# kfirc1503/generative-audio

Hardware: AMD Instinct MI355X
Metric: spectrogram-frames/sec, NPPC K=5 FullSubNet+ train step (higher is better)
Workload: dtype bf16

## Files before the change

generative-audio_amd/csrc/mfma_tile.h:

```cpp
#pragma once
#include "common.h"

enum { EPI_PLAIN = 0, EPI_PRELU_STATS = 1, EPI_RESIDUAL = 2, EPI_RELU = 3, EPI_PLAIN_F32 = 4, EPI_MASK_POS = 5, EPI_RESIDUAL_GN = 6 };

struct GemmArgs {
  const void* A; long lda; long strideA;
  const void* B; long ldb; long strideB;
  void* C; long ldc; long strideC;
  const float* bias; long strideBias;
  const void* res; long ldres; long strideRes;
  const float* slope; long strideSlope;
  double* stats; long strideStats;
  int R, N, K;
  int Tp, Tv;
  int Nv;
  int relu_in;
  int ksplit;
  const float* gnv; long strideGnv;
  double gcnt; float geps;
  int staged;
  float* colpart; long strideColpart;
};

struct ConvArgs {
// ... 61 lines not shown
    f[0] = lo.x; f[1] = lo.y; f[2] = lo.z; f[3] = lo.w; f[4] = hi.x; f[5] = hi.y; f[6] = hi.z; f[7] = hi.w;
    return f;
  }
}

template <typename T, int BN> struct NtStage {
  u32x4 a0, a1, a2, a3, b0, b1, b2, b3;
  __device__ __forceinline__ void load(const T* pa, long lda, const T* pb, long ldb) {
    a0 = *reinterpret_cast<const u32x4*>(pa);
    a1 = *reinterpret_cast<const u32x4*>(pa + 32 * lda);
    a2 = *reinterpret_cast<const u32x4*>(pa + 64 * lda);
    a3 = *reinterpret_cast<const u32x4*>(pa + 96 * lda);
    b0 = *reinterpret_cast<const u32x4*>(pb);
    b1 = *reinterpret_cast<const u32x4*>(pb + 32 * ldb);
    if constexpr (BN == 128) {
      b2 = *reinterpret_cast<const u32x4*>(pb + 64 * ldb);
      b3 = *reinterpret_cast<const u32x4*>(pb + 96 * ldb);
    }
  }
  __device__ __forceinline__ void store(unsigned char* p) const {
    *reinterpret_cast<u32x4*>(p) = a0;
    *reinterpret_cast<u32x4*>(p + 32 * 128) = a1;
    *reinterpret_cast<u32x4*>(p + 64 * 128) = a2;
    *reinterpret_cast<u32x4*>(p + 96 * 128) = a3;
    *reinterpret_cast<u32x4*>(p + 128 * 128) = b0;
    *reinterpret_cast<u32x4*>(p + 128 * 128 + 32 * 128) = b1;
    if constexpr (BN == 128) {
      *reinterpret_cast<u32x4*>(p + 128 * 128 + 64 * 128) = b2;
      *reinterpret_cast<u32x4*>(p + 128 * 128 + 96 * 128) = b3;
    }
  }
};

template <typename T, int BN, typename I, typename AOf, typename BOf>
__device__ __forceinline__ void nt_lds_mainloop(f32x4 (&acc)[4][BN / 32], unsigned char* lds, I nstage, long lda, long ldb,
                                                AOf a_of, BOf b_of, int relu_in) {
  typedef typename Frag<T>::type frag;
  constexpr int KS = (128 / (int)sizeof(T)) / 32;
  constexpr int NJ = BN / 32;
  constexpr int STAGE = (128 + BN) * 128;
  const int tid = threadIdx.x, lane = tid & 63, wave = tid >> 6, n = lane & 15, q = lane >> 4;
  const int wm = wave >> 1, wn = wave & 1;
  const int srow = tid >> 3, sc = tid & 7;
  const int soff = srow * 128 + ((sc ^ (srow & 7)) << 4);
  NtStage<T, BN> st;
#pragma unroll
  for (int i = 0; i < 4; ++i)
#pragma unroll
    for (int j = 0; j < NJ; ++j) acc[i][j] = f32x4{0.f, 0.f, 0.f, 0.f};
  {
    const T* pa = a_of((I)0);
    st.load(pa, lda, b_of((I)0), ldb);
  }
  st.store(lds + soff);
  __syncthreads();
  for (I s = 0; s < nstage; ++s) {
    const int buf = (int)(s & 1);
    const unsigned char* ta = lds + buf * STAGE;
    if (s + 1 < nstage) {
      const T* pa = a_of(s + 1);
      st.load(pa, lda, b_of(s + 1), ldb);
    }
#pragma unroll
    for (int ks = 0; ks < KS; ++ks) {
      frag af[4], bf[NJ];
#pragma unroll
      for (int i = 0; i < 4; ++i) {
        af[i] = lds_frag<T>(ta, wm * 64 + 16 * i + n, ks, q);
        if (relu_in) af[i] = relu_frag<T>(af[i]);
      }
#pragma unroll
      for (int j = 0; j < NJ; ++j) bf[j] = lds_frag<T>(ta + 128 * 128, wn * (BN / 2) + 16 * j + n, ks, q);
#pragma unroll
      for (int i = 0; i < 4; ++i)
#pragma unroll
        for (int j = 0; j < NJ; ++j) acc[i][j] = mma16(af[i], bf[j], acc[i][j]);
    }
    if (s + 1 < nstage) st.store(lds + (buf ^ 1) * STAGE + soff);
    __syncthreads();
  }
}

template <typename T, typename AOf, typename BOf>
__device__ __forceinline__ void nt_reg_mainloop(f32x4 (&acc)[2][4], int nk, long lda, long ldb, AOf a_of, BOf b_of, int relu_in) {
  typedef typename Frag<T>::type frag;
#pragma unroll
  for (int mi = 0; mi < 2; ++mi)
#pragma unroll
    for (int ni = 0; ni < 4; ++ni) acc[mi][ni] = f32x4{0.f, 0.f, 0.f, 0.f};
  frag a0[2], b0[4], a1[2], b1[4];
  auto ld = [&](frag(&a)[2], frag(&b)[4], int kk) {
    const T* pa = a_of(kk);
    const T* pb = b_of(kk);
#pragma unroll
    for (int mi = 0; mi < 2; ++mi) a[mi] = load_frag<T>(pa + (long)16 * mi * lda);
#pragma unroll
    for (int ni = 0; ni < 4; ++ni) b[ni] = load_frag<T>(pb + (long)16 * ni * ldb);
  };
  auto mm = [&](frag(&a)[2], frag(&b)[4]) {
    if (relu_in) {
#pragma unroll
      for (int mi = 0; mi < 2; ++mi) a[mi] = relu_frag<T>(a[mi]);
    }
#pragma unroll
    for (int mi = 0; mi < 2; ++mi)
#pragma unroll
      for (int ni = 0; ni < 4; ++ni) acc[mi][ni] = mma16(a[mi], b[ni], acc[mi][ni]);
  };
  ld(a0, b0, 0);
  int kk = 0;
#pragma unroll 1
  for (; kk + 2 < nk; kk += 2) {
// ... 5 lines not shown
  if (kk + 1 < nk) {
    ld(a1, b1, kk + 1);
    mm(a0, b0);
    mm(a1, b1);
  } else {
    mm(a0, b0);
  }
}

template <typename T, int EPI> struct NtEpilogue {
  const GemmArgs& g;
  const float* bias;
  const float* gnv = nullptr;
  const T* res = nullptr;
  T* C;
  float* Cf;
  float slope = 0.f, gn_rstd = 1.f, gn_mr = 0.f;
  __device__ __forceinline__ NtEpilogue(const GemmArgs& g_, int z, int m0) : g(g_) {
    C = reinterpret_cast<T*>(g.C) + (size_t)blockIdx.z * g.strideC;
    Cf = reinterpret_cast<float*>(g.C) + (size_t)blockIdx.z * g.strideC;
    bias = g.bias ? g.bias + (size_t)z * g.strideBias : nullptr;
    if (EPI == EPI_PRELU_STATS) slope = g.slope[(size_t)z * g.strideSlope];
    if (EPI == EPI_RESIDUAL_GN) {
      const double* st = g.stats + (size_t)z * g.strideStats + (size_t)(m0 / g.Tp) * 2;
      const double m = st[0] / g.gcnt, var = st[1] / g.gcnt - m * m;
      gn_rstd = (float)(1.0 / sqrt((var > 0 ? var : 0) + (double)g.geps));
      gn_mr = (float)m * gn_rstd;
      gnv = g.gnv + (size_t)z * g.strideGnv;
    }
    if (EPI == EPI_RESIDUAL || EPI == EPI_RESIDUAL_GN || EPI == EPI_MASK_POS) res = reinterpret_cast<const T*>(g.res) + (size_t)z * g.strideRes;
  }
  __device__ __forceinline__ float col_bias(int col) const {
    const bool cvalid = col < g.Nv;
    float bv = (bias && cvalid) ? bias[col] : 0.f;
    if (EPI == EPI_RESIDUAL_GN && cvalid) bv -= gn_mr * gnv[col];
    return bv;
  }
  __device__ __forceinline__ float act(float a, float bv) const {
    float v = (EPI == EPI_RESIDUAL_GN ? gn_rstd * a : a) + bv;
    if (EPI == EPI_PRELU_STATS) v = v > 0.f ? v : slope * v;
    if (EPI == EPI_RELU) v = fmaxf(v, 0.f);
    return v;
  }
  __device__ __forceinline__ float put(float a, float bv, int row, int col) const {
    const bool valid = col < g.Nv && (row % g.Tp) < g.Tv;
    float v = act(a, bv);
    if (EPI == EPI_RESIDUAL || EPI == EPI_RESIDUAL_GN) v += to_f32<T>(res[(size_t)row * g.ldres + col]);
    if (EPI == EPI_MASK_POS) {
      if (!(to_f32<T>(res[(size_t)row * g.ldres + col]) > 0.f)) v = 0.f;
    }
    if (!valid) v = 0.f;
    if (EPI == EPI_PLAIN_F32) {
      Cf[(size_t)row * g.ldc + col] = v;
      return v;
    }
    const T o = from_f32<T>(v);
    C[(size_t)row * g.ldc + col] = o;
    return to_f32<T>(o);
  }
};

__device__ __forceinline__ float mul_unfused(float a, float b) {
#pragma clang fp contract(off)
  return a * b;
}


template <typename T, int MI, int NJ>
__device__ __forceinline__ void conv_epilogue(const ConvArgs& g, const f32x4 (&acc)[MI][NJ], long row0, int col0, float (&st1)[NJ],
                                              float (&st2)[NJ]) {
  T* C = reinterpret_cast<T*>(g.C);
#pragma unroll
  for (int i = 0; i < MI; ++i)
#pragma unroll
    for (int r = 0; r < 4; ++r) {
      const long row = row0 + 16 * i + r;
      if (!interior(row, g.P, g.H, g.W)) continue;
#pragma unroll
// ... 45 lines not shown
```

generative-audio_amd/csrc/tcn.hip:

```cpp
#include <cstdlib>
#include "common.h"
#include "mfma_tile.h"
#include "nppc_hip.h"

namespace {


template <typename T, int EPI>
__global__ __launch_bounds__(256) void gemm_nt_kernel(GemmArgs g) {
  const int ks = g.ksplit > 1 ? g.ksplit : 1;
  const int z = blockIdx.z / ks, ksl = blockIdx.z % ks;
  const T* A = reinterpret_cast<const T*>(g.A) + (size_t)z * g.strideA + (size_t)ksl * g.K;
  const T* B = reinterpret_cast<const T*>(g.B) + (size_t)z * g.strideB + (size_t)ksl * g.K;
  const int lane = threadIdx.x & 63, wave = threadIdx.x >> 6, n = lane & 15, q = lane >> 4;
  const int r0 = blockIdx.x * 128 + wave * 32, c0 = blockIdx.y * 64;
  const T* ap = A + (size_t)(r0 + n) * g.lda + 8 * q;
  const T* bp = B + (size_t)(c0 + n) * g.ldb + 8 * q;
  f32x4 acc[2][4];
  nt_reg_mainloop<T>(acc, g.K / 32, g.lda, g.ldb, [&](int kk) { return ap + 32 * kk; }, [&](int kk) { return bp + 32 * kk; },
                     g.relu_in);

  const NtEpilogue<T, EPI> ep(g, z, blockIdx.x * 128);
  float s1 = 0.f, s2 = 0.f;
#pragma unroll
  for (int ni = 0; ni < 4; ++ni) {
    const int col = c0 + 16 * ni + n;
    const float bv = ep.col_bias(col);
#pragma unroll
    for (int mi = 0; mi < 2; ++mi)
#pragma unroll
      for (int j = 0; j < 4; ++j) {
        const float vo = ep.put(acc[mi][ni][j], bv, r0 + 16 * mi + 4 * q + j, col);
        if (EPI == EPI_PRELU_STATS) {
          s1 += vo;
          s2 += vo * vo;
        }
      }
  }
  if (EPI == EPI_PRELU_STATS) {
    double d1 = wave_sum((double)s1), d2 = wave_sum((double)s2);
    if (lane == 0) {
      double* st = g.stats + (size_t)z * g.strideStats + (size_t)(r0 / g.Tp) * 2;
      atomicAdd(st, d1);
      atomicAdd(st + 1, d2);
    }
  }
}

template <typename T, int EPI, int BN>
__global__ __launch_bounds__(256, 2) void gemm_nt_lds_kernel(GemmArgs g) {
  constexpr int EPC = 16 / (int)sizeof(T);
  constexpr int BK = 8 * EPC;
  constexpr int NJ = BN / 32;
  __shared__ __attribute__((aligned(16))) unsigned char lds[2][(128 + BN) * 128];
  __shared__ double red[2][4];
  const int ks_ = g.ksplit > 1 ? g.ksplit : 1;
  const int z = blockIdx.z / ks_, ksl = blockIdx.z % ks_;
  const int tid = threadIdx.x, lane = tid & 63, wave = tid >> 6, n = lane & 15, q = lane >> 4;
  const int wm = wave >> 1, wn = wave & 1;
  const int m0 = blockIdx.x * 128, n0 = blockIdx.y * BN;
  const int srow = tid >> 3, sc = tid & 7;
  const T* ga = reinterpret_cast<const T*>(g.A) + (size_t)z * g.strideA + (size_t)ksl * g.K + (long)(m0 + srow) * g.lda + sc * EPC;
  const T* gb = reinterpret_cast<const T*>(g.B) + (size_t)z * g.strideB + (size_t)ksl * g.K + (long)(n0 + srow) * g.ldb + sc * EPC;
  const int nstage = g.K / BK;
  f32x4 acc[4][NJ];
  nt_lds_mainloop<T, BN>(acc, &lds[0][0], nstage, g.lda, g.ldb, [&](int s) { return ga + s * BK; }, [&](int s) { return gb + s * BK; },
                         g.relu_in);
  const NtEpilogue<T, EPI> ep(g, z, m0);
  constexpr bool HAS_RES = EPI == EPI_RESIDUAL || EPI == EPI_RESIDUAL_GN || EPI == EPI_MASK_POS;
  constexpr bool STAGED_PLAIN = sizeof(T) == 2 && (EPI == EPI_PLAIN || EPI == EPI_PRELU_STATS || EPI == EPI_RELU);
  if constexpr (HAS_RES || STAGED_PLAIN) {
    if (g.staged) {
      constexpr int LD = BN + 4, VE = 8, CPR = BN / VE;
      constexpr int HALVES = (128 * LD * 4 <= (int)sizeof(lds)) ? 1 : 2;
      constexpr int ROWS = 128 / HALVES;
      float* ot = reinterpret_cast<float*>(&lds[0][0]);
      float csum[VE];
      float t1 = 0.f, t2 = 0.f;
#pragma unroll
      for (int e = 0; e < VE; ++e) csum[e] = 0.f;
      for (int h = 0; h < HALVES; ++h) {
        if (HALVES == 1 || wm == h) {
#pragma unroll
          for (int j = 0; j < NJ; ++j) {
            const int col = n0 + wn * (BN / 2) + 16 * j + n;
            const bool cvalid = col < g.Nv;
            const float bv = ep.col_bias(col);
#pragma unroll
            for (int i = 0; i < 4; ++i)
#pragma unroll
              for (int r = 0; r < 4; ++r) {
                const float pv = ep.act(acc[i][j][r], bv);
                ot[((HALVES == 1 ? wm * 64 : 0) + 16 * i + 4 * q + r) * LD + wn * (BN / 2) + 16 * j + n] = pv;
                if (EPI == EPI_PRELU_STATS) {
                  const int row = m0 + wm * 64 + 16 * i + 4 * q + r;
                  const float vo = (cvalid && (row % g.Tp) < g.Tv) ? to_f32<T>(from_f32<T>(pv)) : 0.f;
                  t1 += vo;
                  t2 += vo * vo;
                }
              }
          }
        }
        __syncthreads();
        for (int c = tid; c < ROWS * CPR; c += 256) {
          const int rl = c / CPR, cc = (c % CPR) * VE;
          const int row = m0 + h * ROWS * (HALVES - 1) + rl, col = n0 + cc;
          const bool rvalid = (row % g.Tp) < g.Tv;
          float v[VE], rv[VE];
          const float4 lo = *reinterpret_cast<const float4*>(ot + rl * LD + cc), hi = *reinterpret_cast<const float4*>(ot + rl * LD + cc + 4);
          v[0] = lo.x; v[1] = lo.y; v[2] = lo.z; v[3] = lo.w; v[4] = hi.x; v[5] = hi.y; v[6] = hi.z; v[7] = hi.w;
          if constexpr (HAS_RES) load8<T>(ep.res + (size_t)row * g.ldres + col, rv);
#pragma unroll
          for (int e = 0; e < VE; ++e) {
            float x = v[e];
            if constexpr (HAS_RES) {
              if (EPI == EPI_MASK_POS) { if (!(rv[e] > 0.f)) x = 0.f; }
              else x += rv[e];
            }
            if (!(rvalid && col + e < g.Nv)) x = 0.f;
            v[e] = x;
            csum[e] += to_f32<T>(from_f32<T>(x));
          }
          store8<T>(reinterpret_cast<T*>(g.C) + (size_t)blockIdx.z * g.strideC + (size_t)row * g.ldc + col, v);
        }
        if (HALVES == 2) __syncthreads();
      }
      if (EPI == EPI_PRELU_STATS) {
        const double d1 = wave_sum((double)t1), d2 = wave_sum((double)t2);
        __syncthreads();
        if (lane == 0) { red[0][wave] = d1; red[1][wave] = d2; }
        __syncthreads();
        if (tid == 0) {
          double* st = g.stats + (size_t)z * g.strideStats + (size_t)(m0 / g.Tp) * 2;
          atomicAdd(st, red[0][0] + red[0][1] + red[0][2] + red[0][3]);
          atomicAdd(st + 1, red[1][0] + red[1][1] + red[1][2] + red[1][3]);
        }
      }
      if (HAS_RES && EPI != EPI_RESIDUAL_GN && g.colpart) {
        __shared__ float cpl[4][BN];
#pragma unroll
        for (int e = 0; e < VE; ++e) {
          float cv = csum[e];
#pragma unroll
          for (int m = CPR; m < 64; m <<= 1) cv += __shfl_xor(cv, m);
          if (lane < CPR) cpl[wave][lane * VE + e] = cv;
        }
        __syncthreads();
        if (tid < BN)
          g.colpart[(size_t)z * g.strideColpart + (size_t)blockIdx.x * g.N + n0 + tid] =
              cpl[0][tid] + cpl[1][tid] + cpl[2][tid] + cpl[3][tid];
      }
      return;
    }
  }
  float s1 = 0.f, s2 = 0.f;
  float cs[NJ];
#pragma unroll
  for (int j = 0; j < NJ; ++j) {
    cs[j] = 0.f;
    const int col = n0 + wn * (BN / 2) + 16 * j + n;
    const float bv = ep.col_bias(col);
#pragma unroll
    for (int i = 0; i < 4; ++i)
#pragma unroll
      for (int r = 0; r < 4; ++r) {
        const float vo = ep.put(acc[i][j][r], bv, m0 + wm * 64 + 16 * i + 4 * q + r, col);
        if (EPI == EPI_RESIDUAL || EPI == EPI_MASK_POS) cs[j] += vo;
        if (EPI == EPI_PRELU_STATS) {
          s1 += vo;
          s2 += vo * vo;
        }
      }
  }
  if constexpr (EPI == EPI_RESIDUAL || EPI == EPI_MASK_POS) {
    if (g.colpart) {
      __shared__ float cpl[2][BN];
#pragma unroll
      for (int j = 0; j < NJ; ++j) {
        float c = cs[j];
        c += __shfl_xor(c, 16);
        c += __shfl_xor(c, 32);
        if (q == 0) cpl[wm][wn * (BN / 2) + 16 * j + n] = c;
      }
      __syncthreads();
      if (tid < BN)
        g.colpart[(size_t)z * g.strideColpart + (size_t)blockIdx.x * g.N + n0 + tid] = cpl[0][tid] + cpl[1][tid];
    }
  }
  if (EPI == EPI_PRELU_STATS) {
    const double d1 = wave_sum((double)s1), d2 = wave_sum((double)s2);
    if (lane == 0) { red[0][wave] = d1; red[1][wave] = d2; }
    __syncthreads();
    if (tid == 0) {
      double* st = g.stats + (size_t)z * g.strideStats + (size_t)(m0 / g.Tp) * 2;
      atomicAdd(st, red[0][0] + red[0][1] + red[0][2] + red[0][3]);
      atomicAdd(st + 1, red[1][0] + red[1][1] + red[1][2] + red[1][3]);
    }
  }
}
// ... 127 lines not shown
  float su = 0.f, sv = 0.f;
  for (int k = threadIdx.x; k < ldd; k += 64) {
    float wg = 0.f;
    if (nn < N && k < K) {
      const float w = W[so + (size_t)nn * K + k];
      wg = gamma[so + k] * w;
      su += beta[so + k] * w;
    }
    const T o = from_f32<T>(wg);
    dst[k] = o;
    sv += to_f32<T>(o);
  }
  su = wave_sum(su);
  sv = wave_sum(sv);
  if (threadIdx.x == 0) {
    u[(size_t)ab * Npad + nn] = nn < N ? su + bias[so + nn] : 0.f;
    v[(size_t)ab * Npad + nn] = sv;
  }
}

}

static int nt_staged_plain() {
  const char* e = getenv("NPPC_NT_STAGED_PLAIN");
  return (e && e[0] == '0') ? 0 : 1;
}

template <typename T, int EPI> static void launch_nt_path(int lds_path, int nz, const GemmArgs& g, hipStream_t s) {
  dim3 grid(g.R / 128, lds_path == 128 ? g.N / 128 : g.N / 64, nz);
  if (lds_path == 128) hipLaunchKernelGGL((gemm_nt_lds_kernel<T, EPI, 128>), grid, dim3(256), 0, s, g);
  else if (lds_path == 64) hipLaunchKernelGGL((gemm_nt_lds_kernel<T, EPI, 64>), grid, dim3(256), 0, s, g);
  else hipLaunchKernelGGL((gemm_nt_kernel<T, EPI>), grid, dim3(256), 0, s, g);
}
template <typename T> static int dispatch_nt_epi(int epi, int lds_path, int nz, const GemmArgs& g, hipStream_t s) {
  switch (epi) {
#define NT_CASE(E) case E: launch_nt_path<T, E>(lds_path, nz, g, s); break;
    NT_CASE(EPI_PLAIN) NT_CASE(EPI_PRELU_STATS) NT_CASE(EPI_RESIDUAL) NT_CASE(EPI_RELU) NT_CASE(EPI_PLAIN_F32) NT_CASE(EPI_MASK_POS)
    NT_CASE(EPI_RESIDUAL_GN)
#undef NT_CASE
    default: return NPPC_EBADARG;
  }
  NPPC_CHECK_LAUNCH();
  return NPPC_OK;
}
static int dispatch_nt(int prec, int epi, int lds_path, int nz, const GemmArgs& g, hipStream_t s) {
  if (prec == NPPC_PREC_BF16) return dispatch_nt_epi<bf16_t>(epi, lds_path, nz, g, s);
  if (prec == NPPC_PREC_F32) return dispatch_nt_epi<float>(epi, lds_path, nz, g, s);
  return NPPC_EBADARG;
}

static int launch_nt(int prec, int epi, const void* A, long lda, long sA, const void* B, long ldb, long sB, void* C, long ldc,
                     long sC, const float* bias, long sBias, const void* res, long ldres, long sRes, const float* slope,
                     long sSlope, double* stats, long sStats, int R, int N, int K, int Tp, int Tv, int Nv, int relu_in,
                     int batch, int ksplit, float* colpart, void* stream) {
  if (!A || !B || !C || R <= 0 || N <= 0 || K <= 0 || batch <= 0) return NPPC_EBADARG;
  if (R % 128 || N % 64 || K % 32 || Tp <= 0 || (Tp % 128) || lda % 8 || ldb % 8) return NPPC_EUNSUPPORTED;
  if (epi == EPI_PRELU_STATS && (!slope || !stats)) return NPPC_EBADARG;
  if ((epi == EPI_RESIDUAL || epi == EPI_MASK_POS) && !res) return NPPC_EBADARG;
  if (epi == EPI_RESIDUAL_GN) return NPPC_EBADARG;
  if (ksplit < 1) ksplit = 1;
  if (ksplit > 1 && (epi != EPI_PLAIN_F32 || bias || stats)) return NPPC_EUNSUPPORTED;
  if (K % (32 * ksplit)) return NPPC_EUNSUPPORTED;
  GemmArgs g{A, lda, sA, B, ldb, sB, C, ldc, sC, bias, sBias, res, ldres, sRes, slope, sSlope, stats, sStats,
             R, N, K / ksplit, Tp, Tv, Nv, relu_in, ksplit, nullptr, 0, 1.0, 0.f,
             ((res ? ldres % 8 == 0
                   : ((epi == EPI_PLAIN || epi == EPI_PRELU_STATS || epi == EPI_RELU) && ksplit == 1 && nt_staged_plain())) &&
              ldc % 8 == 0) ? 1 : 0,
             colpart, (long)(R / 128) * N};
  const int bk = prec == NPPC_PREC_BF16 ? 64 : 32;
  const int lds_path = ((K / ksplit) % bk == 0) ? (N % 128 == 0 ? 128 : 64) : 0;
  if (colpart && (lds_path == 0 || ksplit != 1 || (epi != EPI_RESIDUAL && epi != EPI_MASK_POS))) return NPPC_EUNSUPPORTED;
  return dispatch_nt(prec, epi, lds_path, batch * ksplit, g, (hipStream_t)stream);
}

extern "C" {

int nppc_gemm_nt(int prec, int epi, const void* A, long lda, long sA, const void* B, long ldb, long sB, void* C, long ldc,
                 long sC, const float* bias, long sBias, const void* res, long ldres, long sRes, const float* slope,
                 long sSlope, double* stats, long sStats, int R, int N, int K, int Tp, int Tv, int Nv, int relu_in,
                 int batch, int ksplit, void* stream) {
  return launch_nt(prec, epi, A, lda, sA, B, ldb, sB, C, ldc, sC, bias, sBias, res, ldres, sRes, slope, sSlope, stats, sStats, R, N,
                   K, Tp, Tv, Nv, relu_in, batch, ksplit, nullptr, stream);
}

int nppc_gemm_nt_colsum(int prec, int epi, const void* A, long lda, long sA, const void* B, long ldb, long sB, void* C, long ldc,
                        long sC, const float* bias, long sBias, const void* res, long ldres, long sRes, int R, int N, int K,
                        int Tp, int Tv, int Nv, int batch, float* colpart, void* stream) {
  if (!colpart) return NPPC_EBADARG;
  return launch_nt(prec, epi, A, lda, sA, B, ldb, sB, C, ldc, sC, bias, sBias, res, ldres, sRes, nullptr, 0, nullptr, 0, R, N, K,
                   Tp, Tv, Nv, 0, batch, 1, colpart, stream);
}

int nppc_gemm_nt_gn(int prec, const void* A, long lda, long sA, const void* Wg, long ldb, long sB, void* C, long ldc, long sC,
                    const float* u, const float* v, long sUV, const void* res, long ldres, long sRes, const double* stats,
                    long sStats, double cnt, float eps, int R, int N, int K, int Tp, int Tv, int Nv, int batch, void* stream) {
  if (!A || !Wg || !C || !u || !v || !res || !stats || R <= 0 || N <= 0 || K <= 0 || batch <= 0 || cnt <= 0) return NPPC_EBADARG;
  if (R % 128 || N % 64 || K % 32 || Tp <= 0 || (Tp % 128) || lda % 8 || ldb % 8) return NPPC_EUNSUPPORTED;
  GemmArgs g{A, lda, sA, Wg, ldb, sB, C, ldc, sC, u, sUV, res, ldres, sRes, nullptr, 0, const_cast<double*>(stats), sStats,
             R, N, K, Tp, Tv, Nv, 0, 1, v, sUV, cnt, eps, (ldc % 8 == 0 && ldres % 8 == 0) ? 1 : 0, nullptr, 0};
  const int bk = prec == NPPC_PREC_BF16 ? 64 : 32;
  const int lds_path = (K % bk == 0) ? (N % 128 == 0 ? 128 : 64) : 0;
  return dispatch_nt(prec, EPI_RESIDUAL_GN, lds_path, batch, g, (hipStream_t)stream);
}

int nppc_tcn_pack_sconv(int prec, const float* W, const float* gamma, const float* beta, const float* bias, void* Wg, float* u,
                        float* v, int N, int K, int Npad, int ldd, int n_a, int n_b, long src_stride_a, long src_stride_b,
                        long dst_stride_a, long dst_stride_b, void* stream) {
  if (!W || !gamma || !beta || !bias || !Wg || !u || !v || N > Npad || K > ldd || n_a <= 0 || n_b <= 0 || (long)n_a * n_b > 65535)
    return NPPC_EBADARG;
  LAUNCH_TS(prec, pack_sconv_kernel, dim3(Npad, n_a * n_b), dim3(64), 0, W, gamma, beta, bias, (TT*)Wg, u, v, N, K, Npad, ldd, n_b,
            src_stride_a, src_stride_b, dst_stride_a, dst_stride_b);
  return NPPC_OK;
}

int nppc_tcn_dwconv(int prec, const void* in, void* out, const double* st1, double* st2, const float* gamma,
                    const float* beta, const float* wd, const float* bd, const float* slope2, int B, int Cc, int ld, int Tp,
                    int Tv, int dil, float eps, long sAct, long sSt, long sP, int batch, void* stream) {
  if (!in || !out || !st1 || !st2 || Cc % 8 || Cc / 8 > 256) return NPPC_EBADARG;
  LAUNCH_T(prec, dwconv_kernel, dim3(ceil_div(Tp, DW_FRAMES), B, batch), (const TT*)in, (TT*)out, st1, st2, gamma, beta, wd, bd,
           slope2, Cc, ld, Tp, Tv, dil, eps, sAct, sSt, sP);
  return NPPC_OK;
}

int nppc_tcn_gn_apply(int prec, const void* in, void* out, const double* st, const float* gamma, const float* beta, int B,
                      int Cc, int ld, int Tp, int Tv, float eps, long sAct, long sSt, long sP, int batch, void* stream) {
  if (!in || !out || !st || Cc % 8) return NPPC_EBADARG;
  LAUNCH_T(prec, gn_apply_kernel, dim3(ceil_div((long)Tv * (Cc / 8), 256), B, batch), (const TT*)in, (TT*)out, st, gamma, beta, Cc,
           ld, Tp, Tv, eps, sAct, sSt, sP);
  return NPPC_OK;
}

int nppc_pack_matrix(int prec, const float* src, void* dst, int N, int K, int Npad, int ldd, int transpose, void* stream) {
  if (!src || !dst || N > Npad || K > ldd) return NPPC_EBADARG;
  const long total = (long)Npad * ldd;
// ... 592 lines not shown
```

generative-audio_amd/nppc_audio/_hip.py:

```python
import ctypes
import os
import threading

import torch

_HERE = os.path.dirname(os.path.abspath(__file__))
LIB_PATH = os.path.join(_HERE, "libnppc_hip.so")

PREC_BF16 = 0
PREC_F32 = 1
_ERR = {1: "bad argument", 2: "kernel launch failed", 3: "unsupported shape/configuration"}

_lib = None

c_p = ctypes.c_void_p
c_i = ctypes.c_int
c_l = ctypes.c_long
c_f = ctypes.c_float


def lib():
    global _lib
    if _lib is None:
        if not os.path.exists(LIB_PATH):
# ... 94 lines not shown
    "nppc_lstm2_fwd_ws": [I, P, P, P, P, P, P, P, P, P, P, P, P, P, P, P, I, L, I, I, I, P],
    "nppc_lstm2_coop_bwd_packed_elems": [PL],
    "nppc_lstm2_coop_bwd_pack": [P, P, P, P, I, P, P, P],
    "nppc_lstm2_bwd_coop": [P, P, P, P, P, P, P, P, P, P, P, L, P, L, I, I, P],
    "nppc_lstm2_coop_bwd2_packed_elems": [PL],
    "nppc_lstm2_coop_bwd2_pack": [P, P, P, P, I, P, P, P],
    "nppc_lstm2_bwd_coop2": [P, P, P, P, P, P, P, P, P, P, P, L, P, L, I, I, P],
    "nppc_lstm2_bwd_coop2_head": [P, P, P, P, P, P, P, P, P, P, P, P, L, P, L, I, I, P],
    "nppc_lstm2_coop_bwd4_sizes": [L, PL, PL, PL],
    "nppc_lstm2_coop_bwd4_pack": [P, P, P, P, I, P, P, P],
    "nppc_lstm2_bwd_coop4": [P, P, P, P, P, P, P, P, P, P, P, P, P, L, P, L, I, I, P],
    "nppc_head_dy_gather": [P, P, L, I, I, I, I, P],
    "nppc_sb_head_bwd_w": [I, P, P, P, P, L, I, I, I, I, I, P],
    "nppc_lstm2_bwd_packed_elems": [I, I, PL, PL],
    "nppc_lstm2_pack_weights_bwd": [I, P, P, P, P, I, I, P, P, P],
    "nppc_lstm2_bwd": [I, P, P, P, P, P, P, P, P, P, P, L, I, I, I, P],
    "nppc_stft": [P, P, P, P, I, I, I, I, P],
    "nppc_dropband": [P, P, I, I, I, I, I, P],
    "nppc_cirm_build_compress": [P, P, P, P, P, I, I, I, I, F, P],
    "nppc_cirm_decompress_apply_conj": [P, P, P, P, P, P, P, I, I, I, P],
    "nppc_cirm_decompress_apply": [P, P, P, P, P, P, P, I, I, I, P],
    "nppc_istft": [P, P, P, I, I, I, I, I, P],
    "nppc_rowsum": [P, P, L, I, P],
    "nppc_tsse_fwd": [P, P, P, P, P, P, P, P, I, I, I, P, P, P, P, P, P, P, P, P, P, P, P, I, I, I, I, P],
    "nppc_tsse_fwd_maps": [I, P, I, P, P, P, P, P, P, P, I, I, I, P, P, P, P, P, P, L, P, P, P, P, P, P, P, L, I, I, I, I, I, I, P],
    "nppc_tsse_bwd_maps": [I, P, L, P, I, P, P, P, P, I, I, I, P, P, P, L, P, P, P, P, P, P, P, P, P, P, P, P, P, P, P, P, P, P,
                           I, I, I, I, I, I, P],
    "nppc_scale_transpose": [I, P, P, P, I, I, I, I, I, I, P],
    "nppc_gemm_nt": [I, I, P, L, L, P, L, L, P, L, L, P, L, P, L, L, P, L, P, L, I, I, I, I, I, I, I, I, I, P],
    "nppc_tcn_mid_bwd_part_elems": [I, I, I, I, PL],
    "nppc_tcn_mid_bwd": [I, P, P, P, P, P, P, P, P, P, P, P, P, P, P, P, P, P, P, P, P, P, P, P, P, P, P, I, I, I, P,
                         I, I, I, I, I, F, L, L, L, I, I, P],
    "nppc_tcn_mid_bwd_finish": [P, L, P, L, I, I, I, P, P, P, P, P, P, P, P, P, P, I, I, L, L, I, I, P],
    "nppc_gemm_nt_colsum": [I, I, P, L, L, P, L, L, P, L, L, P, L, P, L, L, I, I, I, I, I, I, I, P, P],
    "nppc_gemm_nt_gn": [I, P, L, L, P, L, L, P, L, L, P, P, L, P, L, L, P, L, D, F, I, I, I, I, I, I, I, P],
    "nppc_tcn_pack_sconv": [I, P, P, P, P, P, P, P, I, I, I, I, I, I, L, L, L, L, P],
    "nppc_gemm_nt_splitk": [I, P, L, P, L, P, L, I, I, L, I, P],
    "nppc_gemm_tn_splitk": [P, L, P, L, P, L, I, I, L, I, P],
    "nppc_gemm_tn_splitk_rowsum": [P, L, P, L, P, L, I, I, L, I, P, P],
    "nppc_gemm_tn_splitk2": [P, L, P, L, I, P, L, I, P, L, I, L, I, P, P],
    "nppc_gemm_tn_splitk_batched": [P, L, L, P, L, L, P, L, L, I, I, L, I, I, P],
    "nppc_gemm_tn_grouped": [P, I, I, I, L, P],
    "nppc_reduce_slabs_t": [P, I, L, L, P, L, I, I, L, L, I, P],
    "nppc_gemm_tn_splitk_taps": [P, L, P, L, P, L, I, I, L, I, I, I, P],
    "nppc_tcn_dwconv": [I, P, P, P, P, P, P, P, P, P, I, I, I, I, I, I, F, L, L, L, I, P],
    "nppc_tcn_gn_apply": [I, P, P, P, P, P, I, I, I, I, I, F, L, L, L, I, P],
    "nppc_pack_matrix": [I, P, P, I, I, I, I, I, P],
    "nppc_pack_matrix_batched": [I, P, P, I, I, I, I, I, I, I, L, L, L, L, P],
    "nppc_subband_mean": [I, P, I, P, I, L, P, P, P, I, I, I, I, I, P],
    "nppc_subband_stage": [I, P, I, P, I, L, P, P, I, I, I, I, I, I, I, I, P],
    "nppc_sb_head": [I, P, P, P, P, L, I, I, I, I, I, P],
    "nppc_gram": [P, P, P, P, P, I, I, L, P],
    "nppc_combine": [P, P, P, P, P, P, P, I, I, L, P],
    "nppc_gs_solve": [P, P, P, I, I, I, P],
    "nppc_gs_bwd_solve": [P, P, P, P, I, I, I, P],
    "nppc_loss_solve": [P, P, P, P, P, P, P, P, P, P, I, I, P],
    "nppc_loss_bwd_coef": [P, P, P, F, F, P, I, I, P],
    "nppc_loss_bwd_coef_dev": [P, P, P, P, F, F, P, I, I, P],
    "nppc_transpose": [I, P, P, I, I, L, L, L, L, I, I, P],
    "nppc_colsum": [I, P, P, I, I, L, L, L, I, P, L, P],
    "nppc_colsum_scratch_elems": [I, I, I, PL],
    "nppc_sb_head_bwd": [I, P, P, P, P, P, P, L, I, I, I, I, I, P],
    "nppc_subband_stage_bwd": [I, P, P, P, P, P, P, I, I, I, I, I, L, I, I, I, P],
    "nppc_subband_unfold_bwd": [I, P, P, P, P, P, I, I, I, I, I, I, I, I, P],
    "nppc_reduce_slabs": [P, I, L, L, P, L, I, I, I, I, I, L, L, I, P],
    "nppc_adam_step": [P, P, P, P, L, D, D, D, D, D, I, D, P],
# ... 179 lines not shown
```

include/nppc_hip.h:

```cpp
#ifndef NPPC_HIP_H
#define NPPC_HIP_H
#ifdef __cplusplus
extern "C" {
#endif

int nppc_stft(const float* wave, float* re, float* im, float* mag , int B, int L, int nfft, int hop,
              void* stream);
int nppc_dropband(const float* in, float* out, int B, int C, int F, int T, int G, void* stream);
int nppc_cirm_build_compress(const float* nr, const float* ni, const float* cr, const float* ci, float* out, int B, int F,
                             int T, int G, float eps, void* stream);
int nppc_cirm_decompress_apply_conj(const float* crm, const float* nr, const float* ni, float* dec ,
                                    float* emag, float* ere, float* eim, int B, int F, int T, void* stream);

int nppc_cirm_decompress_apply(const float* crm, const float* nr, const float* ni, float* dec , float* emag,
                               float* ere, float* eim, int B, int F, int T, void* stream);
int nppc_istft(const float* re, const float* im, float* out, int B, int T, int nfft, int hop, int L, void* stream);

int nppc_rowsum(const float* x, double* sums, long R, int T, void* stream);
int nppc_tsse_fwd_maps(int prec, const float* const* maps, int nmaps, double* rowsum, const float* cw0, const float* cb0,
                       const float* cw1, const float* cb1, const float* cw2, const float* cb2, int ks0, int ks1, int ks2,
                       const float* fcw, const float* fcb, const float* w1, const float* b1, const float* w2, const float* b2, long sW,
                       float* scale, float* ns, float* pre, float* sq, float* h1, float* sg, void* X0, long sY, int B, int C, int T,
                       int look_ahead, int Tp, int ld, void* stream);
int nppc_tsse_bwd_ws_elems(int nmaps, int B, int C, int ks0, int ks1, int ks2, long* elems);
int nppc_tsse_bwd_maps(int prec, const void* dX0, long sY, const float* const* maps, int nmaps, const double* rowsum,
                       const float* cw0, const float* cw1, const float* cw2, int ks0, int ks1, int ks2, const float* fcw,
                       const float* w1, const float* w2, long sW, const float* ns, const float* pre, const float* sq,
                       const float* h1, const float* sg, float* ws, float* g_cw0, float* g_cb0, float* g_cw1, float* g_cb1,
                       float* g_cw2, float* g_cb2, float* g_fcw, float* g_fcb, float* g_w1, float* g_b1, float* g_w2, float* g_b2,
                       int B, int C, int T, int look_ahead, int Tp, int ld, void* stream);
int nppc_tsse_fwd(const float* x, const double* rowsum, const float* cw0, const float* cb0, const float* cw1,
                  const float* cb1, const float* cw2, const float* cb2, int ks0, int ks1, int ks2, const float* fcw,
                  const float* fcb, const float* w1, const float* b1, const float* w2, const float* b2, float* scale,
                  float* ns, float* pre, float* sq, float* h1, float* sg, int B, int C, int T, int look_ahead,
                  void* stream);
int nppc_tsse_bwd(int prec, const void* dX0, const float* x, const double* rowsum, const float* cw0, const float* cw1,
                  const float* cw2, int ks0, int ks1, int ks2, const float* fcw, const float* w1, const float* w2,
                  const float* ns, const float* pre, const float* sq, const float* h1, const float* sg, float* dsg_ws,
                  float* g_cw0, float* g_cb0, float* g_cw1, float* g_cb1, float* g_cw2, float* g_cb2, float* g_fcw,
                  float* g_fcb, float* g_w1, float* g_b1, float* g_w2, float* g_b2, int B, int C, int T, int look_ahead, int Tp,
                  int ld, int coff, void* stream);
int nppc_scale_transpose(int prec, const float* x, const float* scale , void* y, int B, int C, int T, int Tp,
                         int ld, int coff, void* stream);

int nppc_gemm_nt(int prec, int epi, const void* A, long lda, long sA, const void* B, long ldb, long sB, void* C, long ldc,
                 long sC, const float* bias, long sBias, const void* res, long ldres, long sRes, const float* slope,
                 long sSlope, double* stats, long sStats, int R, int N, int K, int Tp, int Tv, int Nv, int relu_in,
                 int batch, int ksplit, void* stream);
int nppc_gemm_nt_splitk(int prec, const void* A, long lda, const void* B, long ldb, float* C, long ldc, int M, int N, long K,
                        int ksplit, void* stream);
int nppc_gemm_tn_splitk(const void* A, long lda, const void* B, long ldb, float* C, long ldc, int M, int N, long R, int ksplit,
                        void* stream);
int nppc_gemm_tn_splitk_rowsum(const void* A, long lda, const void* B, long ldb, float* C, long ldc, int M, int N, long R,
                               int ksplit, float* rowsum, void* stream);
int nppc_gemm_tn_splitk2(const void* A, long lda, const void* B1, long ldb1, int N1, const void* B2, long ldb2, int N2, float* C,
                         long ldc, int M, long R, int ksplit, float* rowsum, void* stream);
int nppc_gemm_tn_splitk_batched(const void* A, long lda, long sA, const void* B, long ldb, long sB, float* C, long ldc, long sC,
                                int M, int N, long R, int ksplit, int batch, void* stream);
enum { NPPC_TN_STORE_ASIS = 0, NPPC_TN_STORE_TRANSPOSED = 1 };
typedef struct nppc_tn_problem {
  const void* A; long lda;
  const void* B; long ldb;
  float* dst; long dst_ld;
  long nvalid;
  long kind;
} nppc_tn_problem;
int nppc_gemm_tn_grouped(const nppc_tn_problem* table, int nprob, int M, int N, long R, void* stream);
int nppc_gemm_tn_splitk_taps(const void* A, long lda, const void* B, long ldb, float* C, long ldc, int M, int N, long R,
                             int ksplit, int Wp, int shift_a, void* stream);
int nppc_pack_matrix(int prec, const float* src, void* dst, int N, int K, int Npad, int ldd, int transpose, void* stream);
int nppc_pack_matrix_batched(int prec, const float* src, void* dst, int N, int K, int Npad, int ldd, int transpose, int n_a,
                             int n_b, long src_stride_a, long src_stride_b, long dst_stride_a, long dst_stride_b, void* stream);
int nppc_tcn_dwconv(int prec, const void* in, void* out, const double* st1, double* st2, const float* gamma,
                    const float* beta, const float* wd, const float* bd, const float* slope2, int B, int Cc, int ld, int Tp,
                    int Tv, int dil, float eps, long sAct, long sSt, long sP, int batch, void* stream);
int nppc_tcn_gn_apply(int prec, const void* in, void* out, const double* st, const float* gamma, const float* beta, int B,
                      int Cc, int ld, int Tp, int Tv, float eps, long sAct, long sSt, long sP, int batch, void* stream);
int nppc_tcn_gn_bwd(int prec, const void* dA, const void* y, const double* st, const float* gamma, const float* slope,
                    double* S, void* dpre, float* dgamma, float* dbeta, float* dslope, int B, int Cc, int Tp, int Tv, float eps,
                    long sAct, long sSt, long sP, int batch, void* stream);
int nppc_tcn_dwconv_bwd(int prec, const void* du, const void* y1, const double* st1, const float* gamma, const float* beta,
// ... 464 lines not shown
```

Before: 258,900.

## Single-buffer LDS for bf16 NT GEMM to raise occupancy, restructure staged epilogue

Result: faster. 261,800 (median of 6 runs) (+1.1%).

```diff
diff --git a/generative-audio_amd/csrc/mfma_tile.h b/generative-audio_amd/csrc/mfma_tile.h
--- a/generative-audio_amd/csrc/mfma_tile.h
+++ b/generative-audio_amd/csrc/mfma_tile.h
@@ -117,11 +117,32 @@
   }
 };
 
+template <typename T, int BN>
+__device__ __forceinline__ void nt_lds_stage_mma(f32x4 (&acc)[4][BN / 32], const unsigned char* ta, int wm, int wn, int n, int q,
+                                                 int relu_in) {
+  typedef typename Frag<T>::type frag;
+  constexpr int KS = (128 / (int)sizeof(T)) / 32;
+  constexpr int NJ = BN / 32;
+#pragma unroll
+  for (int ks = 0; ks < KS; ++ks) {
+    frag af[4], bf[NJ];
+#pragma unroll
+    for (int i = 0; i < 4; ++i) {
+      af[i] = lds_frag<T>(ta, wm * 64 + 16 * i + n, ks, q);
+      if (relu_in) af[i] = relu_frag<T>(af[i]);
+    }
+#pragma unroll
+    for (int j = 0; j < NJ; ++j) bf[j] = lds_frag<T>(ta + 128 * 128, wn * (BN / 2) + 16 * j + n, ks, q);
+#pragma unroll
+    for (int i = 0; i < 4; ++i)
+#pragma unroll
+      for (int j = 0; j < NJ; ++j) acc[i][j] = mma16(af[i], bf[j], acc[i][j]);
+  }
+}
+
 template <typename T, int BN, typename I, typename AOf, typename BOf>
 __device__ __forceinline__ void nt_lds_mainloop(f32x4 (&acc)[4][BN / 32], unsigned char* lds, I nstage, long lda, long ldb,
                                                 AOf a_of, BOf b_of, int relu_in) {
-  typedef typename Frag<T>::type frag;
-  constexpr int KS = (128 / (int)sizeof(T)) / 32;
   constexpr int NJ = BN / 32;
   constexpr int STAGE = (128 + BN) * 128;
   const int tid = threadIdx.x, lane = tid & 63, wave = tid >> 6, n = lane & 15, q = lane >> 4;
@@ -146,23 +167,43 @@
       const T* pa = a_of(s + 1);
       st.load(pa, lda, b_of(s + 1), ldb);
     }
-#pragma unroll
-    for (int ks = 0; ks < KS; ++ks) {
-      frag af[4], bf[NJ];
-#pragma unroll
-      for (int i = 0; i < 4; ++i) {
-        af[i] = lds_frag<T>(ta, wm * 64 + 16 * i + n, ks, q);
-        if (relu_in) af[i] = relu_frag<T>(af[i]);
-      }
-#pragma unroll
-      for (int j = 0; j < NJ; ++j) bf[j] = lds_frag<T>(ta + 128 * 128, wn * (BN / 2) + 16 * j + n, ks, q);
-#pragma unroll
-      for (int i = 0; i < 4; ++i)
-#pragma unroll
-        for (int j = 0; j < NJ; ++j) acc[i][j] = mma16(af[i], bf[j], acc[i][j]);
-    }
+    nt_lds_stage_mma<T, BN>(acc, ta, wm, wn, n, q, relu_in);
     if (s + 1 < nstage) st.store(lds + (buf ^ 1) * STAGE + soff);
     __syncthreads();
+  }
+}
+
+template <typename T, int BN, typename I, typename AOf, typename BOf>
+__device__ __forceinline__ void nt_lds_mainloop_1buf(f32x4 (&acc)[4][BN / 32], unsigned char* lds, I nstage, long lda, long ldb,
+                                                     AOf a_of, BOf b_of, int relu_in) {
+  constexpr int NJ = BN / 32;
+  const int tid = threadIdx.x, lane = tid & 63, wave = tid >> 6, n = lane & 15, q = lane >> 4;
+  const int wm = wave >> 1, wn = wave & 1;
+  const int srow = tid >> 3, sc = tid & 7;
+  const int soff = srow * 128 + ((sc ^ (srow & 7)) << 4);
+  NtStage<T, BN> st;
+#pragma unroll
+  for (int i = 0; i < 4; ++i)
+#pragma unroll
+    for (int j = 0; j < NJ; ++j) acc[i][j] = f32x4{0.f, 0.f, 0.f, 0.f};
+  {
+    const T* pa = a_of((I)0);
+    st.load(pa, lda, b_of((I)0), ldb);
+  }
+  st.store(lds + soff);
+  __syncthreads();
+  for (I s = 0; s < nstage; ++s) {
+    const bool more = s + 1 < nstage;
+    if (more) {
+      const T* pa = a_of(s + 1);
+      st.load(pa, lda, b_of(s + 1), ldb);
+    }
+    nt_lds_stage_mma<T, BN>(acc, lds, wm, wn, n, q, relu_in);
+    __syncthreads();
+    if (more) {
+      st.store(lds + soff);
+      __syncthreads();
+    }
   }
 }
 
@@ -234,8 +275,10 @@
   }
   __device__ __forceinline__ float col_bias(int col) const {
     const bool cvalid = col < g.Nv;
-    float bv = (bias && cvalid) ? bias[col] : 0.f;
-    if (EPI == EPI_RESIDUAL_GN && cvalid) bv -= gn_mr * gnv[col];
+    const int cl = cvalid ? col : 0;
+    float bv = bias ? bias[cl] : 0.f;
+    if (EPI == EPI_RESIDUAL_GN) bv -= gn_mr * gnv[cl];
+    if (!cvalid) bv = 0.f;
     return bv;
   }
   __device__ __forceinline__ float act(float a, float bv) const {
@@ -244,8 +287,9 @@
     if (EPI == EPI_RELU) v = fmaxf(v, 0.f);
     return v;
   }
-  __device__ __forceinline__ float put(float a, float bv, int row, int col) const {
-    const bool valid = col < g.Nv && (row % g.Tp) < g.Tv;
+  __device__ __forceinline__ float put(float a, float bv, int row, int col) const { return put(a, bv, row, col, (row % g.Tp) < g.Tv); }
+  __device__ __forceinline__ float put(float a, float bv, int row, int col, bool rvalid) const {
+    const bool valid = col < g.Nv && rvalid;
     float v = act(a, bv);
     if (EPI == EPI_RESIDUAL || EPI == EPI_RESIDUAL_GN) v += to_f32<T>(res[(size_t)row * g.ldres + col]);
     if (EPI == EPI_MASK_POS) {
diff --git a/generative-audio_amd/csrc/tcn.hip b/generative-audio_amd/csrc/tcn.hip
--- a/generative-audio_amd/csrc/tcn.hip
+++ b/generative-audio_amd/csrc/tcn.hip
@@ -47,12 +47,19 @@
   }
 }
 
+template <typename T, int EPI, int BN> constexpr int nt_lds_wg_per_cu() {
+  if (sizeof(T) != 2) return 2;
+  if (BN == 64) return 4;
+  return (EPI == EPI_RESIDUAL || EPI == EPI_MASK_POS || EPI == EPI_RESIDUAL_GN) ? 2 : 3;
+}
+
 template <typename T, int EPI, int BN>
-__global__ __launch_bounds__(256, 2) void gemm_nt_lds_kernel(GemmArgs g) {
+__global__ __launch_bounds__(256, (nt_lds_wg_per_cu<T, EPI, BN>())) void gemm_nt_lds_kernel(GemmArgs g) {
   constexpr int EPC = 16 / (int)sizeof(T);
   constexpr int BK = 8 * EPC;
   constexpr int NJ = BN / 32;
-  __shared__ __attribute__((aligned(16))) unsigned char lds[2][(128 + BN) * 128];
+  constexpr int NBUF = sizeof(T) == 2 ? 1 : 2;
+  __shared__ __attribute__((aligned(16))) unsigned char lds[NBUF][(128 + BN) * 128];
   __shared__ double red[2][4];
   const int ks_ = g.ksplit > 1 ? g.ksplit : 1;
   const int z = blockIdx.z / ks_, ksl = blockIdx.z % ks_;
@@ -64,48 +71,62 @@
   const T* gb = reinterpret_cast<const T*>(g.B) + (size_t)z * g.strideB + (size_t)ksl * g.K + (long)(n0 + srow) * g.ldb + sc * EPC;
   const int nstage = g.K / BK;
   f32x4 acc[4][NJ];
-  nt_lds_mainloop<T, BN>(acc, &lds[0][0], nstage, g.lda, g.ldb, [&](int s) { return ga + s * BK; }, [&](int s) { return gb + s * BK; },
-                         g.relu_in);
+  if constexpr (NBUF == 1)
+    nt_lds_mainloop_1buf<T, BN>(acc, &lds[0][0], nstage, g.lda, g.ldb, [&](int s) { return ga + s * BK; },
+                                [&](int s) { return gb + s * BK; }, g.relu_in);
+  else
+    nt_lds_mainloop<T, BN>(acc, &lds[0][0], nstage, g.lda, g.ldb, [&](int s) { return ga + s * BK; }, [&](int s) { return gb + s * BK; },
+                           g.relu_in);
   const NtEpilogue<T, EPI> ep(g, z, m0);
+  const int tp0 = m0 % g.Tp;
   constexpr bool HAS_RES = EPI == EPI_RESIDUAL || EPI == EPI_RESIDUAL_GN || EPI == EPI_MASK_POS;
   constexpr bool STAGED_PLAIN = sizeof(T) == 2 && (EPI == EPI_PLAIN || EPI == EPI_PRELU_STATS || EPI == EPI_RELU);
   if constexpr (HAS_RES || STAGED_PLAIN) {
     if (g.staged) {
       constexpr int LD = BN + 4, VE = 8, CPR = BN / VE;
-      constexpr int HALVES = (128 * LD * 4 <= (int)sizeof(lds)) ? 1 : 2;
-      constexpr int ROWS = 128 / HALVES;
+      constexpr int ROWS = 128 * LD * 4 <= (int)sizeof(lds) ? 128 : 64 * LD * 4 <= (int)sizeof(lds) ? 64 : 32;
+      constexpr int PASSES = 128 / ROWS;
+      static_assert(ROWS * LD * 4 <= (int)sizeof(lds) && (ROWS * CPR) % 256 == 0 && 256 % CPR == 0, "epilogue passes");
       float* ot = reinterpret_cast<float*>(&lds[0][0]);
       float csum[VE];
       float t1 = 0.f, t2 = 0.f;
 #pragma unroll
       for (int e = 0; e < VE; ++e) csum[e] = 0.f;
-      for (int h = 0; h < HALVES; ++h) {
-        if (HALVES == 1 || wm == h) {
-#pragma unroll
-          for (int j = 0; j < NJ; ++j) {
-            const int col = n0 + wn * (BN / 2) + 16 * j + n;
-            const bool cvalid = col < g.Nv;
-            const float bv = ep.col_bias(col);
-#pragma unroll
-            for (int i = 0; i < 4; ++i)
-#pragma unroll
-              for (int r = 0; r < 4; ++r) {
-                const float pv = ep.act(acc[i][j][r], bv);
-                ot[((HALVES == 1 ? wm * 64 : 0) + 16 * i + 4 * q + r) * LD + wn * (BN / 2) + 16 * j + n] = pv;
-                if (EPI == EPI_PRELU_STATS) {
-                  const int row = m0 + wm * 64 + 16 * i + 4 * q + r;
-                  const float vo = (cvalid && (row % g.Tp) < g.Tv) ? to_f32<T>(from_f32<T>(pv)) : 0.f;
-                  t1 += vo;
-                  t2 += vo * vo;
-                }
-              }
+#pragma unroll
+      for (int j = 0; j < NJ; ++j) {
+        const int col = n0 + wn * (BN / 2) + 16 * j + n;
+        const bool cvalid = col < g.Nv;
+        const float bv = ep.col_bias(col);
+#pragma unroll
+        for (int i = 0; i < 4; ++i)
+#pragma unroll
+          for (int r = 0; r < 4; ++r) {
+            const float pv = ep.act(acc[i][j][r], bv);
+            acc[i][j][r] = pv;
+            if (EPI == EPI_PRELU_STATS) {
+              const unsigned keep = (cvalid && tp0 + wm * 64 + 16 * i + 4 * q + r < g.Tv) ? ~0u : 0u;
+              const float vo = __uint_as_float(__float_as_uint(to_f32<T>(from_f32<T>(pv))) & keep);
+              t1 += vo;
+              t2 += vo * vo;
+            }
           }
+      }
+#pragma unroll
+      for (int h = 0; h < PASSES; ++h) {
+#pragma unroll
+        for (int i = 0; i < 4; ++i) {
+          if ((wm * 4 + i) / (ROWS / 16) != h) continue;
+#pragma unroll
+          for (int j = 0; j < NJ; ++j)
+#pragma unroll
+            for (int r = 0; r < 4; ++r)
+              ot[(wm * 64 + 16 * i + 4 * q + r - h * ROWS) * LD + wn * (BN / 2) + 16 * j + n] = acc[i][j][r];
         }
         __syncthreads();
         for (int c = tid; c < ROWS * CPR; c += 256) {
           const int rl = c / CPR, cc = (c % CPR) * VE;
-          const int row = m0 + h * ROWS * (HALVES - 1) + rl, col = n0 + cc;
-          const bool rvalid = (row % g.Tp) < g.Tv;
+          const int row = m0 + h * ROWS + rl, col = n0 + cc;
+          const bool rvalid = tp0 + h * ROWS + rl < g.Tv;
           float v[VE], rv[VE];
           const float4 lo = *reinterpret_cast<const float4*>(ot + rl * LD + cc), hi = *reinterpret_cast<const float4*>(ot + rl * LD + cc + 4);
           v[0] = lo.x; v[1] = lo.y; v[2] = lo.z; v[3] = lo.w; v[4] = hi.x; v[5] = hi.y; v[6] = hi.z; v[7] = hi.w;
@@ -123,11 +144,10 @@
           }
           store8<T>(reinterpret_cast<T*>(g.C) + (size_t)blockIdx.z * g.strideC + (size_t)row * g.ldc + col, v);
         }
-        if (HALVES == 2) __syncthreads();
+        if (h + 1 < PASSES) __syncthreads();
       }
       if (EPI == EPI_PRELU_STATS) {
         const double d1 = wave_sum((double)t1), d2 = wave_sum((double)t2);
-        __syncthreads();
         if (lane == 0) { red[0][wave] = d1; red[1][wave] = d2; }
         __syncthreads();
         if (tid == 0) {
@@ -164,7 +184,8 @@
     for (int i = 0; i < 4; ++i)
 #pragma unroll
       for (int r = 0; r < 4; ++r) {
-        const float vo = ep.put(acc[i][j][r], bv, m0 + wm * 64 + 16 * i + 4 * q + r, col);
+        const int rl = wm * 64 + 16 * i + 4 * q + r;
+        const float vo = ep.put(acc[i][j][r], bv, m0 + rl, col, tp0 + rl < g.Tv);
         if (EPI == EPI_RESIDUAL || EPI == EPI_MASK_POS) cs[j] += vo;
         if (EPI == EPI_PRELU_STATS) {
           s1 += vo;
@@ -358,6 +379,11 @@
   else if (lds_path == 64) hipLaunchKernelGGL((gemm_nt_lds_kernel<T, EPI, 64>), grid, dim3(256), 0, s, g);
   else hipLaunchKernelGGL((gemm_nt_kernel<T, EPI>), grid, dim3(256), 0, s, g);
 }
+static int nt_tile_width(int prec, int N, int kslice) {
+  const int bk = prec == NPPC_PREC_BF16 ? 64 : 32;
+  if (kslice % bk) return 0;
+  return N % 128 == 0 ? 128 : 64;
+}
 template <typename T> static int dispatch_nt_epi(int epi, int lds_path, int nz, const GemmArgs& g, hipStream_t s) {
   switch (epi) {
 #define NT_CASE(E) case E: launch_nt_path<T, E>(lds_path, nz, g, s); break;
@@ -393,8 +419,7 @@
                    : ((epi == EPI_PLAIN || epi == EPI_PRELU_STATS || epi == EPI_RELU) && ksplit == 1 && nt_staged_plain())) &&
               ldc % 8 == 0) ? 1 : 0,
              colpart, (long)(R / 128) * N};
-  const int bk = prec == NPPC_PREC_BF16 ? 64 : 32;
-  const int lds_path = ((K / ksplit) % bk == 0) ? (N % 128 == 0 ? 128 : 64) : 0;
+  const int lds_path = nt_tile_width(prec, N, K / ksplit);
   if (colpart && (lds_path == 0 || ksplit != 1 || (epi != EPI_RESIDUAL && epi != EPI_MASK_POS))) return NPPC_EUNSUPPORTED;
   return dispatch_nt(prec, epi, lds_path, batch * ksplit, g, (hipStream_t)stream);
 }
@@ -407,6 +432,14 @@
                  int batch, int ksplit, void* stream) {
   return launch_nt(prec, epi, A, lda, sA, B, ldb, sB, C, ldc, sC, bias, sBias, res, ldres, sRes, slope, sSlope, stats, sStats, R, N,
                    K, Tp, Tv, Nv, relu_in, batch, ksplit, nullptr, stream);
+}
+
+int nppc_gemm_nt_tile(int prec, int N, int K, int ksplit, int* bn) {
+  if (!bn || (prec != NPPC_PREC_BF16 && prec != NPPC_PREC_F32) || N <= 0 || K <= 0) return NPPC_EBADARG;
+  if (ksplit < 1) ksplit = 1;
+  if (N % 64 || K % (32 * ksplit)) return NPPC_EUNSUPPORTED;
+  *bn = nt_tile_width(prec, N, K / ksplit);
+  return NPPC_OK;
 }
 
 int nppc_gemm_nt_colsum(int prec, int epi, const void* A, long lda, long sA, const void* B, long ldb, long sB, void* C, long ldc,
@@ -424,8 +457,7 @@
   if (R % 128 || N % 64 || K % 32 || Tp <= 0 || (Tp % 128) || lda % 8 || ldb % 8) return NPPC_EUNSUPPORTED;
   GemmArgs g{A, lda, sA, Wg, ldb, sB, C, ldc, sC, u, sUV, res, ldres, sRes, nullptr, 0, const_cast<double*>(stats), sStats,
              R, N, K, Tp, Tv, Nv, 0, 1, v, sUV, cnt, eps, (ldc % 8 == 0 && ldres % 8 == 0) ? 1 : 0, nullptr, 0};
-  const int bk = prec == NPPC_PREC_BF16 ? 64 : 32;
-  const int lds_path = (K % bk == 0) ? (N % 128 == 0 ? 128 : 64) : 0;
+  const int lds_path = nt_tile_width(prec, N, K);
   return dispatch_nt(prec, EPI_RESIDUAL_GN, lds_path, batch, g, (hipStream_t)stream);
 }
 
diff --git a/generative-audio_amd/nppc_audio/_hip.py b/generative-audio_amd/nppc_audio/_hip.py
--- a/generative-audio_amd/nppc_audio/_hip.py
+++ b/generative-audio_amd/nppc_audio/_hip.py
@@ -150,6 +150,7 @@
     "nppc_tcn_mid_bwd": [I, P, P, P, P, P, P, P, P, P, P, P, P, P, P, P, P, P, P, P, P, P, P, P, P, P, P, I, I, I, P,
                          I, I, I, I, I, F, L, L, L, I, I, P],
     "nppc_tcn_mid_bwd_finish": [P, L, P, L, I, I, I, P, P, P, P, P, P, P, P, P, P, I, I, L, L, I, I, P],
+    "nppc_gemm_nt_tile": [I, I, I, I, PI],
     "nppc_gemm_nt_colsum": [I, I, P, L, L, P, L, L, P, L, L, P, L, P, L, L, I, I, I, I, I, I, I, P, P],
     "nppc_gemm_nt_gn": [I, P, L, L, P, L, L, P, L, L, P, P, L, P, L, L, P, L, D, F, I, I, I, I, I, I, I, P],
     "nppc_tcn_pack_sconv": [I, P, P, P, P, P, P, P, I, I, I, I, I, I, L, L, L, L, P],
diff --git a/include/nppc_hip.h b/include/nppc_hip.h
--- a/include/nppc_hip.h
+++ b/include/nppc_hip.h
@@ -47,6 +47,7 @@
                  long sC, const float* bias, long sBias, const void* res, long ldres, long sRes, const float* slope,
                  long sSlope, double* stats, long sStats, int R, int N, int K, int Tp, int Tv, int Nv, int relu_in,
                  int batch, int ksplit, void* stream);
+int nppc_gemm_nt_tile(int prec, int N, int K, int ksplit, int* bn);
 int nppc_gemm_nt_splitk(int prec, const void* A, long lda, const void* B, long ldb, float* C, long ldc, int M, int N, long K,
                         int ksplit, void* stream);
 int nppc_gemm_tn_splitk(const void* A, long lda, const void* B, long ldb, float* C, long ldc, int M, int N, long R, int ksplit,
```
